# zhengyk19/vit-rpe-rope

Hardware: AMD Instinct MI355X
Metric: train images/sec, CIFAR-10 ViT d=192 L=6 H=6 (higher is better)
Workload: dtype bf16; 1 GPU; CIFAR-10-shaped 32x32 patch4 ViT d=192 L=6 H=6, --pos_encoding rope-axial theta=100, bf16, full train step (fwd+CE+bwd+AdamW), random-init weights; per_gpu_batch=512, global_batch=512, parallelism=dp1, hip_graph=True

## Files before the change

include/vitpe_debug.h:

```cpp
#ifndef VITPE_DEBUG_H
#define VITPE_DEBUG_H
#include "vitpe.h"
#ifdef __cplusplus
extern "C" {
#endif

int vitpe_selftest_mma(int dtype, const void* A, const void* Bt, const void* Brow, float* C_row,
                       float* C_tr, vitpe_stream_t stream);

int vitpe_debug_attn_occupancy(int which);
int vitpe_debug_wgrad_census(int dtype, const vitpe_wgrad_problem* problems, int nprob, unsigned long long* census,
                             vitpe_stream_t stream);
int vitpe_debug_attn_census(const void* xn, const void* wqkv, void* out, const float* cos, const float* sin,
                            int B, unsigned long long* census, vitpe_stream_t stream);
int vitpe_debug_attn32_census(const void* xn, const void* wqkv_wide, void* out, const float* cos, const float* sin,
                              int B, unsigned long long* census, int exp, vitpe_stream_t stream);
int vitpe_debug_tail2_census(const void* attn_out, const void* x_in, const void* Wp_packed, const float* bp,
                             const float* gamma, const float* beta, void* x_mid, float* mean2, float* rstd2,
                             void* xn_out, const void* W1_packed, const float* b1, const void* W2_packed,
                             const float* b2, void* gp_out, void* h_out, void* out, float* mean_out, float* rstd_out,
                             int M, int HID, unsigned long long* census, int exp, vitpe_stream_t stream);
int vitpe_debug_set_gemm2d_mt(int mt);
int vitpe_debug_set_wgrad_wide(int on);
int vitpe_debug_read_bw(const void* src, long long bytes, int depth, int workgroups, unsigned* sink, vitpe_stream_t stream);
#ifdef __cplusplus
}
#endif
#endif
```

vit-rpe-rope_amd/csrc/attn.hip:

```cpp
#include "attn_common.h"
#include <stdlib.h>
#include <type_traits>

namespace vitpe {

template <typename T, typename C, int KM, int NTH = 384>
VITPE_DEV void stage_tokens(const AttnArgs& a, int b, T* xs, T* hbuf, int hbuf_elems, float* s_tab, float* s_coef,
                            int tid, int nthreads, bool stage_tables) {
  constexpr int CHN = CH<T>::n;
  constexpr int DCH = C::LDX / CHN;
  constexpr int D = C::DD;
  const int N = C::ntok(a);
  const T* xg = reinterpret_cast<const T*>(a.xn) + (size_t)b * N * D;
  const Chunk16 zero = {0u, 0u, 0u, 0u};
  constexpr int TOTAL = C::NP * DCH;
  constexpr int ITERS = (TOTAL + NTH - 1) / NTH;
  Chunk16 v[ITERS];
#pragma unroll
  for (int it = 0; it < ITERS; ++it) {
    const int q = tid + it * nthreads, row = q / DCH, cc = q % DCH;
    v[it] = zero;
    if (q < TOTAL && row < N && cc * CHN < D) v[it] = *reinterpret_cast<const Chunk16*>(xg + (size_t)row * D + cc * CHN);
  }
  if (a.ln_gamma != nullptr) {
// ... 340 lines not shown
    f32x4 o[NT];
#pragma unroll
    for (int dt = 0; dt < NT; ++dt) o[dt] = z4;
#pragma unroll
    for (int sc = 0; sc < SC; ++sc) {
      const Frag<T> bp = acc_to_frag<T>(s[2 * sc], (2 * sc + 1 < MT) ? s[(2 * sc + 1 < MT) ? 2 * sc + 1 : 0] : z4);
#pragma unroll
      for (int dt = 0; dt < NT; ++dt) mma(vf[dt][sc], bp, o[dt]);
    }
    const float inv = __builtin_amdgcn_rcpf(l);
    if (sizeof(T) == 2) {
#pragma unroll
      for (int dp = 0; dp < NT; dp += 2) {
        uint32_t lo[2], hi[2];
#pragma unroll
        for (int w2 = 0; w2 < 2; ++w2) {
          bf16x2 pa, pb;
          const f32x4 oa = o[dp] * inv, ob = o[dp + 1] * inv;
          pa[0] = (bf16)oa[2 * w2]; pa[1] = (bf16)oa[2 * w2 + 1];
          pb[0] = (bf16)ob[2 * w2]; pb[1] = (bf16)ob[2 * w2 + 1];
          const auto r = __builtin_amdgcn_permlane16_swap(__builtin_bit_cast(uint32_t, pa), __builtin_bit_cast(uint32_t, pb),
                                                         false, false);
          lo[w2] = r[0]; hi[w2] = r[1];
        }
        const int f0 = 16 * (dp + (g & 1)) + 8 * (g >> 1);
        if (it < MT - 1 || i < N)
          *reinterpret_cast<Chunk16*>(outp + (size_t)i * D + f0) = (Chunk16){lo[0], lo[1], hi[0], hi[1]};
      }
    } else if (it < MT - 1 || i < N) {
#pragma unroll
      for (int dt = 0; dt < NT; ++dt)
        st4(outp + (size_t)i * D + 16 * dt + 4 * g, o[dt][0] * inv, o[dt][1] * inv, o[dt][2] * inv, o[dt][3] * inv);
    }
  }
  stamp(6);
}

template <typename T, typename C, int NTH>
VITPE_DEV void stage_rows_plain(const T* src, T* dst, int ld, int N, int tid) {
  constexpr int CHN = CH<T>::n, D = C::DD, CPRW = D / CHN, RPP = NTH / CPRW, ITERS = C::NP / RPP;
  const int cc = tid % CPRW, r0 = tid / CPRW;
  const Chunk16 zero = {0u, 0u, 0u, 0u};
  Chunk16 v[ITERS];
#pragma unroll
  for (int it = 0; it < ITERS; ++it) {
    const int row = r0 + it * RPP;
    v[it] = *reinterpret_cast<const Chunk16*>(src + (size_t)min(row, N - 1) * D + cc * CHN);
    if (row >= N) v[it] = zero;
  }
#pragma unroll
  for (int it = 0; it < ITERS; ++it) *reinterpret_cast<Chunk16*>(dst + (r0 + it * RPP) * ld + cc * CHN) = v[it];
}

template <int HD, int D, int MT, int KM, int NTOK, int IPW, bool LNF, bool MIXED, int PDEG = 7>
__global__ __launch_bounds__(64 * (D / HD) * IPW, 3) void attn_bwd_reg_kernel(AttnArgs a) {
  using T = bf16;
  using C = AttnCfg<T, HD, D, MT, 1, NTOK>;
  constexpr int NT = C::NT, KS = C::KS, HC = C::HC, SC = C::SC, NTH = 64 * C::H;
  static_assert(NT == 2 && HC == 1, "head dimension 32");
  constexpr int CSLD = HD / 2 + 8;
  constexpr int FRAG = 64 * 8;
  constexpr int XS_ELEMS = IPW * C::NP * C::LDX, DOS_ELEMS = IPW * C::H * MT * FRAG;
  __shared__ __attribute__((aligned(16))) T xs_all[XS_ELEMS > DOS_ELEMS ? XS_ELEMS : DOS_ELEMS];
  __shared__ __attribute__((aligned(16))) T qs_all[IPW * C::H * MT * FRAG];
  __shared__ __attribute__((aligned(16))) float s_tab[KM == KM_RELATIVE ? C::H * C::TABLD : 4];
  __shared__ __attribute__((aligned(16))) float s_coef[KM == KM_POLY ? C::PESZ : 4];
  __shared__ __attribute__((aligned(16))) float s_cos[KM == KM_ROPE ? C::NP * CSLD : 4];
  __shared__ __attribute__((aligned(16))) float s_sin[KM == KM_ROPE ? C::NP * CSLD : 4];
  __shared__ __attribute__((aligned(16))) float s_stat[IPW * C::H * 2 * C::NP];
  __shared__ float s_dtab[KM == KM_RELATIVE ? C::H * C::TABLD : 4];
  __shared__ float s_dcoef[C::H * (C::MAXDEG + 1)];
  __shared__ float s_dfreq[2 * C::H * (HD / 2)];

  const int N = C::ntok(a), P = N - 1;
  const int lane = threadIdx.x & 63;
  const int wave_all = __builtin_amdgcn_readfirstlane(threadIdx.x >> 6);
  const int img = wave_all / C::H, h = wave_all % C::H;
  const int b_raw = blockIdx.x * IPW + img;
  const bool live = b_raw < a.B;
  const int b = live ? b_raw : a.B - 1;
  const int tid_img = threadIdx.x % NTH;
  T* const xs = xs_all + img * C::NP * C::LDX;
  T* const qsw = qs_all + wave_all * MT * FRAG + lane * 8;
  T* const dsw = xs_all + wave_all * MT * FRAG + lane * 8;
  float* const lse_w = s_stat + (img * C::H + h) * 2 * C::NP;
  float* const del_w = lse_w + C::NP;
  float* const dtab_i = s_dtab;
  float* const dcoef_i = s_dcoef;
  float* const dfreq_i = s_dfreq;
  const int c = lane & 15, g = lane >> 4;
  const f32x4 z4 = {0.f, 0.f, 0.f, 0.f};
  constexpr bool mixed = (KM == KM_ROPE) && MIXED;

  const T* const Wh = reinterpret_cast<const T*>(a.wqkv) + ((size_t)h * 3 * NT * KS * 64 + lane) * 8;
  auto wload = [&](Frag<T> (&w)[NT][KS], int mat) {
#pragma unroll
    for (int nt = 0; nt < NT; ++nt)
#pragma unroll
      for (int ks = 0; ks < KS; ++ks) w[nt][ks] = ld_frag(Wh + (size_t)((mat * NT + nt) * KS + ks) * 64 * 8);
  };
  Frag<T> w[NT][KS];
  wload(w, 2);
  stage_tokens_fwd<T, C, KM, NTH, LNF>(a, b, xs, s_tab, s_coef, tid_img, false, IPW == 1 || img == 0);
  if (KM == KM_ROPE && !mixed) {
    constexpr int F4 = HD / 8;
    for (int q = threadIdx.x; q < C::NP * F4; q += NTH * IPW) {
      const int f4 = q % F4, row = q / F4;
      f32x4 cv = {1.f, 1.f, 1.f, 1.f}, sv = {0.f, 0.f, 0.f, 0.f};
      if (row >= 1 && row < N) {
        cv = *reinterpret_cast<const f32x4*>(a.cos + (size_t)(row - 1) * (HD / 2) + 4 * f4);
        sv = *reinterpret_cast<const f32x4*>(a.sin + (size_t)(row - 1) * (HD / 2) + 4 * f4);
      }
      *reinterpret_cast<f32x4*>(&s_cos[row * CSLD + 4 * f4]) = cv;
      *reinterpret_cast<f32x4*>(&s_sin[row * CSLD + 4 * f4]) = sv;
    }
  }
  if (KM == KM_RELATIVE)
    for (int q = threadIdx.x; q < C::H * C::TABLD; q += NTH * IPW) s_dtab[q] = 0.f;
  for (int q = threadIdx.x; q < C::H * (C::MAXDEG + 1); q += NTH * IPW) s_dcoef[q] = 0.f;
  for (int q = threadIdx.x; q < 2 * C::H * (HD / 2); q += NTH * IPW) s_dfreq[q] = 0.f;
  __syncthreads();

  const T* const xrow = xs + c * C::LDX + 8 * g;
  const unsigned hoff = mixed ? (unsigned)(h * P * (HD / 2)) : 0u;
  auto cs_vec = [&](int tok, int f, f32x4& cv, f32x4& sv) {
    if (!mixed) {
      cv = *reinterpret_cast<const f32x4*>(&s_cos[tok * CSLD + f]);
      sv = *reinterpret_cast<const f32x4*>(&s_sin[tok * CSLD + f]);
    } else {
      const bool ok = tok >= 1 && tok < N;
      const unsigned o = hoff + (unsigned)((min(max(tok, 1), N - 1) - 1) * (HD / 2) + f);
      const f32x4 cg = *reinterpret_cast<const f32x4*>(a.cos + o), sg = *reinterpret_cast<const f32x4*>(a.sin + o);
      cv = ok ? cg : (f32x4){1.f, 1.f, 1.f, 1.f};
      sv = ok ? sg : z4;
    }
  };
  auto proj_sw = [&](int tt, bool rope, float sc, Frag<T>& dst) {
    Frag<T> xf[KS];
#pragma unroll
    for (int ks = 0; ks < KS; ++ks) xf[ks] = ld_frag(xrow + 16 * tt * C::LDX + 32 * ks);
    __builtin_amdgcn_sched_barrier(0);
    f32x4 acc[NT] = {z4, z4};
#pragma unroll
    for (int ks = 0; ks < KS; ++ks)
#pragma unroll
      for (int nt = 0; nt < NT; ++nt) mma(w[nt][ks], xf[ks], acc[nt]);
    __builtin_amdgcn_sched_barrier(0);
    if (KM == KM_ROPE && rope) {
      f32x4 cv, sv;
      cs_vec(16 * tt + c, 4 * g, cv, sv);
      const f32x4 x1 = acc[0], x2 = acc[1];
      acc[0] = x1 * cv - x2 * sv;
      acc[1] = x1 * sv + x2 * cv;
    }
    dst = acc_to_frag<T>(acc[0] * sc, acc[1] * sc);
    asm volatile("" : "+v"(dst.v));
  };
  Frag<T> e0, e1;
#pragma unroll
  for (int t = 0; t < 8; ++t) {
    e0.v[t] = (bf16)((t < 4 && 4 * g + t == c) ? 1.0f : 0.0f);
    e1.v[t] = (bf16)((t >= 4 && 4 * g + t - 4 == c) ? 1.0f : 0.0f);
  }
  auto transpose_pair = [&](const Frag<T>& fa, const Frag<T>* fb, Frag<T>& d0, Frag<T>& d1) {
    f32x4 a0 = z4, a1 = z4, b0 = z4, b1 = z4;
    mma(fa, e0, a0);
    mma(fa, e1, a1);
    if (fb != nullptr) { mma(*fb, e0, b0); mma(*fb, e1, b1); }
    d0 = acc_to_frag<T>(a0, b0);
    d1 = acc_to_frag<T>(a1, b1);
  };

  const float qsc = a.scale * LOG2E;
  Frag<T> vkf[MT], kf[MT];
#pragma unroll
  for (int tt = 0; tt < MT; ++tt) proj_sw(tt, false, 1.0f, vkf[tt]);
  wload(w, 1);
  __builtin_amdgcn_sched_barrier(0);
#pragma unroll
  for (int tt = 0; tt < MT; ++tt) proj_sw(tt, true, 1.0f, kf[tt]);
  wload(w, 0);
  __builtin_amdgcn_sched_barrier(0);
#pragma unroll
  for (int tt = 0; tt < MT; ++tt) {
    Frag<T> qf;
    proj_sw(tt, true, qsc, qf);
    *reinterpret_cast<bf16x8*>(qsw + tt * FRAG) = qf.v;
  }
  __syncthreads();
  if (!live) return;
  {
    const T* dog = reinterpret_cast<const T*>(a.dout) + (size_t)b * N * D + h * HD;
    Frag<T> df[MT];
#pragma unroll
    for (int tt = 0; tt < MT; ++tt) {
      const int tok = 16 * tt + c;
      bf16x4 lo = {(bf16)0.f, (bf16)0.f, (bf16)0.f, (bf16)0.f}, hi = lo;
      if (tok < N) {
        lo = *reinterpret_cast<const bf16x4*>(dog + (size_t)tok * D + 4 * g);
        hi = *reinterpret_cast<const bf16x4*>(dog + (size_t)tok * D + 16 + 4 * g);
      }
      df[tt].v = __builtin_shufflevector(lo, hi, 0, 1, 2, 3, 4, 5, 6, 7);
    }
#pragma unroll
    for (int tt = 0; tt < MT; ++tt) *reinterpret_cast<bf16x8*>(dsw + tt * FRAG) = df[tt].v;
  }
  auto qf_load = [&](int tt) { Frag<T> f; f.v = *reinterpret_cast<const bf16x8*>(qsw + tt * FRAG); return f; };
  auto dof_load = [&](int tt) { Frag<T> f; f.v = *reinterpret_cast<const bf16x8*>(dsw + tt * FRAG); return f; };
  Frag<T> ktf[NT][SC];
#pragma unroll
  for (int scx = 0; scx < SC; ++scx)
    transpose_pair(kf[2 * scx], (2 * scx + 1 < MT) ? &kf[(2 * scx + 1 < MT) ? 2 * scx + 1 : 0] : nullptr, ktf[0][scx], ktf[1][scx]);

  T* const dqg = reinterpret_cast<T*>(a.out) + (size_t)b * N * 3 * D + h * HD;
  auto store_pair = [&](T* rowp, const f32x4& o0, const f32x4& o1, bool ok) {
    uint32_t lo[2], hi[2];
#pragma unroll
    for (int w2 = 0; w2 < 2; ++w2) {
      bf16x2 pa, pb;
      pa[0] = (bf16)o0[2 * w2]; pa[1] = (bf16)o0[2 * w2 + 1];
      pb[0] = (bf16)o1[2 * w2]; pb[1] = (bf16)o1[2 * w2 + 1];
      const auto r = __builtin_amdgcn_permlane16_swap(__builtin_bit_cast(uint32_t, pa), __builtin_bit_cast(uint32_t, pb), false, false);
      lo[w2] = r[0]; hi[w2] = r[1];
    }
    const int f0 = 16 * (g & 1) + 8 * (g >> 1);
    if (ok) *reinterpret_cast<Chunk16*>(rowp + f0) = (Chunk16){lo[0], lo[1], hi[0], hi[1]};
  };

  float cacc[PDEG + 1];
#pragma unroll
  for (int k = 0; k <= PDEG; ++k) cacc[k] = 0.f;
#pragma unroll
  for (int it = 0; it < MT; ++it) {
    __builtin_amdgcn_sched_barrier(0);
    const int i = 16 * it + c;
    const Frag<T> dof = dof_load(it), qfi = qf_load(it);
    f32x4 s[MT], dp[MT];
    float m = -1e30f;
    typedef __attribute__((ext_vector_type(4))) unsigned u32x4;
    const unsigned xyi = (KM == KM_POLY) ? reinterpret_cast<const unsigned*>(s_coef + C::H * C::PBLD)[i] : 0u;
    const float* const ptab = s_coef + (a.coeff_per_head ? h : 0) * C::PBLD;
    const bool qcls = (it == 0) && (c == 0);
#pragma unroll
    for (int jt = 0; jt < MT; ++jt) {
      s[jt] = z4;
      mma(kf[jt], qfi, s[jt]);
      dp[jt] = z4;
      mma(vkf[jt], dof, dp[jt]);
      const u32x4 xyj = (KM == KM_POLY) ? *reinterpret_cast<const u32x4*>(s_coef + C::H * C::PBLD + 16 * jt + 4 * g) : (u32x4){0u, 0u, 0u, 0u};
#pragma unroll
      for (int r = 0; r < 4; ++r) {
        const int j = 16 * jt + 4 * g + r;
        float v = s[jt][r];
        if (KM == KM_RELATIVE) v += pe_bias2<C, KM>(a, s_tab, s_coef, h, i, j, N);
        if (KM == KM_POLY) {
          const float bv = ptab[__builtin_amdgcn_sad_u8(xyi, xyj[r], 0u)];
          const bool cls = qcls || (jt == 0 && r == 0 && g == 0);
          v += cls ? 0.f : bv;
        }
        if (jt == MT - 1) v = (j < N) ? v : -1e30f;
        s[jt][r] = v;
        m = fmaxf(m, v);
      }
    }
    m = xg_max(m);
    float l = 0.f;
#pragma unroll
    for (int jt = 0; jt < MT; ++jt)
#pragma unroll
      for (int r = 0; r < 4; ++r) { const float p = __builtin_amdgcn_exp2f(s[jt][r] - m); s[jt][r] = p; l += p; }
    l = xg_sum(l);
    const float inv = __builtin_amdgcn_rcpf(l);
    float dl = 0.f;
#pragma unroll
    for (int jt = 0; jt < MT; ++jt)
#pragma unroll
      for (int r = 0; r < 4; ++r) { s[jt][r] *= inv; dl += s[jt][r] * dp[jt][r]; }
    dl = xg_sum(dl);
    if (g == 0) { lse_w[i] = m + __builtin_amdgcn_logf(l); del_w[i] = dl; }
    const bool qvalid = (it < MT - 1) || (i < N);
    float tacc[PDEG + 1];
#pragma unroll
    for (int k = 0; k <= PDEG; ++k) tacc[k] = 0.f;
#pragma unroll
    for (int jt = 0; jt < MT; ++jt) {
      if (KM == KM_POLY) __builtin_amdgcn_sched_barrier(0);
      const u32x4 xyj = (KM == KM_POLY) ? *reinterpret_cast<const u32x4*>(s_coef + C::H * C::PBLD + 16 * jt + 4 * g) : (u32x4){0u, 0u, 0u, 0u};
#pragma unroll
      for (int r = 0; r < 4; ++r) {
        const int j = 16 * jt + 4 * g + r;
        const bool valid = qvalid && ((jt < MT - 1) || (j < N));
        const float ds = valid ? s[jt][r] * (dp[jt][r] - dl) : 0.f;
        dp[jt][r] = ds;
        if (KM == KM_POLY) {
          const float dsk = (jt == 0 && r == 0) ? (g == 0 ? 0.f : ds) : ds;
          const float x = (float)__builtin_amdgcn_sad_u8(xyi, xyj[r], 0u);
          float pw = x;
          tacc[0] += dsk;
#pragma unroll
          for (int k = 1; k <= PDEG; ++k) { tacc[k] = fmaf(dsk, pw, tacc[k]); if (k < PDEG) pw *= x; }
        }
      }
    }
    if (KM == KM_POLY) {
      const float qm = (it == 0 && c == 0) ? 0.f : 1.f;
#pragma unroll
      for (int k = 0; k <= PDEG; ++k) {
        cacc[k] = fmaf(qm, tacc[k], cacc[k]);
        asm volatile("" : "+v"(cacc[k]));
      }
    }
    if (KM == KM_RELATIVE) {
#pragma unroll
      for (int jt = 0; jt < MT; ++jt) {
        float d0, d1;
        tile_diag_sums(dp[jt], lane, d0, d1);
        const int idx0 = 16 * (it - jt) + c + N - 1;
        if (g == 0) {
          if (idx0 >= 0 && idx0 <= 2 * N - 2) atomicAdd(&dtab_i[h * C::TABLD + idx0], d0);
          if (c >= 1 && idx0 - 16 >= 0 && idx0 - 16 <= 2 * N - 2) atomicAdd(&dtab_i[h * C::TABLD + idx0 - 16], d1);
        }
      }
    }
    f32x4 dqa[NT] = {z4, z4};
#pragma unroll
    for (int scx = 0; scx < SC; ++scx) {
      const Frag<T> bs = acc_to_frag<T>(dp[2 * scx], (2 * scx + 1 < MT) ? dp[(2 * scx + 1 < MT) ? 2 * scx + 1 : 0] : z4);
#pragma unroll
      for (int dt = 0; dt < NT; ++dt) mma(ktf[dt][scx], bs, dqa[dt]);
    }
    if (mixed) {
      const bool tok_ok = i >= 1 && i < N;
      f32x4 dph;
#pragma unroll
      for (int r = 0; r < 4; ++r) dph[r] = dqa[1][r] * (float)qfi.v[r] - dqa[0][r] * (float)qfi.v[4 + r];
      mixed_freq_grad_tile(dfreq_i, dph, i, tok_ok, 16 * it, h, C::H, P, a.grid, HD / 2, 4 * g, LN2, lane);
    }
    if (KM == KM_ROPE) {
      f32x4 cv, sv;
      cs_vec(min(i, C::NP - 1), 4 * g, cv, sv);
      const f32x4 d1 = dqa[0], d2 = dqa[1];
      dqa[0] = d1 * cv + d2 * sv;
      dqa[1] = d2 * cv - d1 * sv;
    }
    store_pair(dqg + (size_t)i * 3 * D, dqa[0] * a.scale, dqa[1] * a.scale, qvalid);
  }

  if (KM == KM_POLY) {
#pragma unroll
    for (int k = 0; k <= PDEG; ++k)
      if (k <= a.degree) {
        const float t = wave_sum(cacc[k]);
        if (lane == 0) atomicAdd(&dcoef_i[(a.coeff_per_head ? h : 0) * (C::MAXDEG + 1) + k], t);
      }
  }
  Frag<T> qtf[NT][SC], dotf[NT][SC];
  __builtin_amdgcn_sched_barrier(0);
#pragma unroll
  for (int scx = 0; scx < SC; ++scx) {
    const bool two = 2 * scx + 1 < MT;
    const Frag<T> qa = qf_load(2 * scx), qb = qf_load(two ? 2 * scx + 1 : 0);
    transpose_pair(qa, two ? &qb : nullptr, qtf[0][scx], qtf[1][scx]);
    const Frag<T> da = dof_load(2 * scx), db = dof_load(two ? 2 * scx + 1 : 0);
    transpose_pair(da, two ? &db : nullptr, dotf[0][scx], dotf[1][scx]);
  }
  __builtin_amdgcn_s_waitcnt(0xC07F);

#pragma unroll
  for (int jt = 0; jt < MT; ++jt) {
    __builtin_amdgcn_sched_barrier(0);
    const int j = 16 * jt + c;
    const bool kvalid = (jt < MT - 1) || (j < N);
    const unsigned xyk = (KM == KM_POLY) ? reinterpret_cast<const unsigned*>(s_coef + C::H * C::PBLD)[j] : 0u;
    const float* const ptab2 = s_coef + (a.coeff_per_head ? h : 0) * C::PBLD;
    const bool kcls = (jt == 0) && (c == 0);
    f32x4 p[MT], ds[MT];
#pragma unroll
    for (int it = 0; it < MT; ++it) {
      const Frag<T> dof = dof_load(it), qfi = qf_load(it);
      p[it] = z4;
      mma(qfi, kf[jt], p[it]);
      ds[it] = z4;
      mma(dof, vkf[jt], ds[it]);
      const f32x4 lse = *reinterpret_cast<const f32x4*>(&lse_w[16 * it + 4 * g]);
      const f32x4 dlv = *reinterpret_cast<const f32x4*>(&del_w[16 * it + 4 * g]);
      typedef __attribute__((ext_vector_type(4))) unsigned u32x4;
      const u32x4 xyq = (KM == KM_POLY) ? *reinterpret_cast<const u32x4*>(s_coef + C::H * C::PBLD + 16 * it + 4 * g) : (u32x4){0u, 0u, 0u, 0u};
#pragma unroll
      for (int r = 0; r < 4; ++r) {
        const int i = 16 * it + 4 * g + r;
        float sv = p[it][r];
        if (KM == KM_RELATIVE) sv += pe_bias2<C, KM>(a, s_tab, s_coef, h, i, j, N);
        if (KM == KM_POLY) {
          const float bv = ptab2[__builtin_amdgcn_sad_u8(xyk, xyq[r], 0u)];
          const bool cls = kcls || (it == 0 && r == 0 && g == 0);
          sv += cls ? 0.f : bv;
        }
        const bool valid = kvalid && ((it < MT - 1) || (i < N));
        const float pv = valid ? __builtin_amdgcn_exp2f(sv - lse[r]) : 0.f;
        p[it][r] = pv;
        ds[it][r] = pv * (ds[it][r] - dlv[r]);
      }
    }
    f32x4 dva[NT] = {z4, z4}, dka[NT] = {z4, z4};
#pragma unroll
    for (int scx = 0; scx < SC; ++scx) {
      const bool two = (2 * scx + 1 < MT);
      const Frag<T> bp = acc_to_frag<T>(p[2 * scx], two ? p[two ? 2 * scx + 1 : 0] : z4);
      const Frag<T> bs = acc_to_frag<T>(ds[2 * scx], two ? ds[two ? 2 * scx + 1 : 0] : z4);
#pragma unroll
      for (int dt = 0; dt < NT; ++dt) {
        mma(dotf[dt][scx], bp, dva[dt]);
        mma(qtf[dt][scx], bs, dka[dt]);
      }
    }
    dka[0] *= LN2; dka[1] *= LN2;
    if (mixed) {
      const bool tok_ok = j >= 1 && j < N;
      f32x4 dph;
#pragma unroll
      for (int r = 0; r < 4; ++r) dph[r] = dka[1][r] * (float)kf[jt].v[r] - dka[0][r] * (float)kf[jt].v[4 + r];
      mixed_freq_grad_tile(dfreq_i, dph, j, tok_ok, 16 * jt, h, C::H, P, a.grid, HD / 2, 4 * g, 1.0f, lane);
    }
    if (KM == KM_ROPE) {
      f32x4 cv, sv;
      cs_vec(min(j, C::NP - 1), 4 * g, cv, sv);
      const f32x4 d1 = dka[0], d2 = dka[1];
      dka[0] = d1 * cv + d2 * sv;
      dka[1] = d2 * cv - d1 * sv;
    }
    store_pair(dqg + (size_t)j * 3 * D + D, dka[0], dka[1], kvalid);
    store_pair(dqg + (size_t)j * 3 * D + 2 * D, dva[0], dva[1], kvalid);
  }

  __syncthreads();
  const int nrun = NTH * min(IPW, a.B - (int)blockIdx.x * IPW);
  if (KM == KM_RELATIVE) {
    for (int q = threadIdx.x; q < C::H * (2 * N - 1); q += nrun) {
      const int hh = q / (2 * N - 1), i = q % (2 * N - 1);
      atomicAdd(a.dtable + q, s_dtab[hh * C::TABLD + i]);
    }
  } else if (KM == KM_POLY) {
    const int nh = a.coeff_per_head ? C::H : 1;
    for (int q = threadIdx.x; q < nh * (a.degree + 1); q += nrun) {
      const int hh = q / (a.degree + 1), k = q % (a.degree + 1);
      atomicAdd(a.dcoeff + q, s_dcoef[hh * (C::MAXDEG + 1) + k]);
    }
  } else if (mixed) {
    for (int q = threadIdx.x; q < 2 * C::H * (HD / 2); q += nrun) atomicAdd(a.dfreqs + q, s_dfreq[q]);
  }
}

template <typename T, int HD, int D, int MT, int HPP, int KM, int NTOK>
__global__ __launch_bounds__(384) void attn_bwd_kernel(AttnArgs a) {
  using C = AttnCfg<T, HD, D, MT, HPP, NTOK>;
  __shared__ __attribute__((aligned(16))) T xs[C::NP * C::LDX];
  __shared__ __attribute__((aligned(16))) T hb[4 * HPP * C::HSZ];
  __shared__ __attribute__((aligned(16))) float s_tab[KM == KM_RELATIVE ? C::H * C::TABLD : 4];
  __shared__ __attribute__((aligned(16))) float s_coef[KM == KM_POLY ? C::PESZ : 4];
  __shared__ __attribute__((aligned(16))) float s_stat[HPP * 2 * C::NP];
  __shared__ float s_dtab[KM == KM_RELATIVE ? C::H * C::TABLD : 4];
  __shared__ float s_dcoef[C::H * (C::MAXDEG + 1)];
  __shared__ float s_dfreq[2 * C::H * (HD / 2)];
  constexpr int SLD = HPP * HD + Pad<T>::elems;
  __shared__ __attribute__((aligned(16))) T s_dq[3 * C::NP * SLD];

  const int N = C::ntok(a);
  const int b = blockIdx.x;
  const int lane = threadIdx.x & 63;
  const int wave = __builtin_amdgcn_readfirstlane(threadIdx.x >> 6);
  const int c = lane & 15, g = lane >> 4;
  const int P = N - 1;
  WFrags<T, C> wf;
  {
    const int hh = wave / 3, mat = wave % 3;
    if (hh < HPP && hh < C::H) load_w<T, C>(a, wf, hh, mat, lane);
  }
  stage_tokens<T, C, KM>(a, b, xs, hb, 4 * HPP * C::HSZ, s_tab, s_coef, threadIdx.x, 384, true);
  if (KM == KM_RELATIVE)
    for (int q = threadIdx.x; q < C::H * C::TABLD; q += 384) s_dtab[q] = 0.f;
  for (int q = threadIdx.x; q < C::H * (C::MAXDEG + 1); q += 384) s_dcoef[q] = 0.f;
  for (int q = threadIdx.x; q < 2 * C::H * (HD / 2); q += 384) s_dfreq[q] = 0.f;
  __syncthreads();

  constexpr int CHN = CH<T>::n;
// ... 257 lines not shown
            *reinterpret_cast<const Chunk16*>(s_dq + (mat * C::NP + row) * SLD + cc * CHN);
      }
    }
  }

  if (KM == KM_RELATIVE) {
    for (int q = threadIdx.x; q < C::H * (2 * N - 1); q += 384) {
      const int h = q / (2 * N - 1), i = q % (2 * N - 1);
      atomicAdd(a.dtable + q, s_dtab[h * C::TABLD + i]);
    }
  } else if (KM == KM_POLY) {
    const int nh = a.coeff_per_head ? C::H : 1;
    for (int q = threadIdx.x; q < nh * (a.degree + 1); q += 384) {
      const int h = q / (a.degree + 1), k = q % (a.degree + 1);
      atomicAdd(a.dcoeff + q, s_dcoef[h * (C::MAXDEG + 1) + k]);
    }
  } else if (mixed) {
    for (int q = threadIdx.x; q < 2 * C::H * (HD / 2); q += 384) atomicAdd(a.dfreqs + q, s_dfreq[q]);
  }
}

template <typename T>
__global__ void pack_qkv_kernel(const float* __restrict__ w, T* __restrict__ dst, int D, int HD) {
  const int NT = HD / 16, KS = D / 32, H = D / HD;
  const long long total = (long long)3 * D * D;
  for (long long idx = (long long)blockIdx.x * blockDim.x + threadIdx.x; idx < total;
       idx += (long long)gridDim.x * blockDim.x) {
    const int e = (int)(idx & 7), l = (int)((idx >> 3) & 63);
    long long blk = idx >> 9;
    const int ks = (int)(blk % KS); blk /= KS;
    const int nt = (int)(blk % NT); blk /= NT;
    const int mat = (int)(blk % 3);
    const int h = (int)(blk / 3);
    if (h >= H) continue;
    const int c = l & 15, g = l >> 4;
    dst[idx] = from_f32<T>(w[(size_t)(mat * D + h * HD + 16 * nt + c) * D + 32 * ks + 8 * g + e]);
  }
}

}

using namespace vitpe;

extern "C" int vitpe_pack_qkv_weights(int dtype, const float* wqkv, void* packed, int D, int HD, hipStream_t stream) {
  VITPE_REQUIRE(wqkv && packed && D > 0 && HD > 0 && D % HD == 0 && HD % 16 == 0 && D % 32 == 0);
  VITPE_REQUIRE(dtype == 0 || dtype == 1);
  const long long total = (long long)3 * D * D;
  const unsigned blocks = (unsigned)min((total + 255) / 256, (long long)2048);
  if (dtype == 1) hipLaunchKernelGGL(pack_qkv_kernel<bf16>, dim3(blocks), dim3(256), 0, stream, wqkv, (bf16*)packed, D, HD);
  else hipLaunchKernelGGL(pack_qkv_kernel<float>, dim3(blocks), dim3(256), 0, stream, wqkv, (float*)packed, D, HD);
  VITPE_CHECK_LAUNCH();
}

template <typename T, int HD, int D, int MT, int HPP, int KM, int NTOK>
static int launch_attn3(bool bwd, const AttnArgs& a, hipStream_t s) {
  constexpr bool REG_BWD = sizeof(T) == 2 && D / HD <= 6;
  if constexpr (REG_BWD) {
    if (bwd) {
      const dim3 grid((a.B + 1) / 2), block(64 * (D / HD) * 2);
      const bool ln = a.ln_gamma != nullptr;
      if constexpr (KM == KM_ROPE) {
        if (a.mode == PE_ROPE_MIXED) {
          if (ln) hipLaunchKernelGGL((attn_bwd_reg_kernel<HD, D, MT, KM, NTOK, 2, true, true>), grid, block, 0, s, a);
          else hipLaunchKernelGGL((attn_bwd_reg_kernel<HD, D, MT, KM, NTOK, 2, false, true>), grid, block, 0, s, a);
          VITPE_CHECK_LAUNCH();
        }
      }
      if constexpr (KM == KM_POLY) {
        if (a.degree <= 3) {
          if (ln) hipLaunchKernelGGL((attn_bwd_reg_kernel<HD, D, MT, KM, NTOK, 2, true, false, 3>), grid, block, 0, s, a);
          else hipLaunchKernelGGL((attn_bwd_reg_kernel<HD, D, MT, KM, NTOK, 2, false, false, 3>), grid, block, 0, s, a);
          VITPE_CHECK_LAUNCH();
        }
      }
      if (ln) hipLaunchKernelGGL((attn_bwd_reg_kernel<HD, D, MT, KM, NTOK, 2, true, false>), grid, block, 0, s, a);
      else hipLaunchKernelGGL((attn_bwd_reg_kernel<HD, D, MT, KM, NTOK, 2, false, false>), grid, block, 0, s, a);
      VITPE_CHECK_LAUNCH();
    }
  }
  if (bwd) {
    if constexpr (!REG_BWD) hipLaunchKernelGGL((attn_bwd_kernel<T, HD, D, MT, HPP, KM, NTOK>), dim3(a.B), dim3(384), 0, s, a);
  } else {
    constexpr int IPW = (sizeof(T) == 2 && D / HD <= 6) ? 2 : 1;
    const dim3 grid((a.B + IPW - 1) / IPW), block(64 * (D / HD) * IPW);
    if (a.ln_gamma != nullptr) hipLaunchKernelGGL((attn_fwd_kernel<T, HD, D, MT, KM, NTOK, IPW, true>), grid, block, 0, s, a);
    else hipLaunchKernelGGL((attn_fwd_kernel<T, HD, D, MT, KM, NTOK, IPW, false>), grid, block, 0, s, a);
  }
  VITPE_CHECK_LAUNCH();
}

template <typename T, int HD, int D, int MT, int HPP, int NTOK>
static int launch_attn2(bool bwd, const AttnArgs& a, hipStream_t s) {
  switch (a.mode) {
    case PE_RELATIVE: return launch_attn3<T, HD, D, MT, HPP, KM_RELATIVE, NTOK>(bwd, a, s);
    case PE_POLY: return launch_attn3<T, HD, D, MT, HPP, KM_POLY, NTOK>(bwd, a, s);
    case PE_ROPE_AXIAL:
    case PE_ROPE_MIXED: return launch_attn3<T, HD, D, MT, HPP, KM_ROPE, NTOK>(bwd, a, s);
    default: return launch_attn3<T, HD, D, MT, HPP, KM_PLAIN, NTOK>(bwd, a, s);
  }
}

template <typename T, int HD, int D, int MT, int HPP>
static int launch_attn(bool bwd, const AttnArgs& a, hipStream_t s) {
  if (a.N == 65) return launch_attn2<T, HD, D, MT, HPP, 65>(bwd, a, s);
  return launch_attn2<T, HD, D, MT, HPP, 0>(bwd, a, s);
}

static int dispatch_attn(bool bwd, int dtype, int D, int HD, const AttnArgs& a, hipStream_t s) {
  const int MT = (a.N + 15) / 16;
  if (HD != 32 || MT != 5) return (int)hipErrorNotSupported;
  if (dtype == 1) {
    if (D == 192) return launch_attn<bf16, 32, 192, 5, 2>(bwd, a, s);
    if (D == 96) return launch_attn<bf16, 32, 96, 5, 2>(bwd, a, s);
// ... 97 lines not shown
```

vit-rpe-rope_amd/vitpe/kernels.py:

```python
from __future__ import annotations

import ctypes
from typing import Optional, Tuple

import torch

from . import _lib as L
from ._lib import check, dtype_code, lib, ptr, require_device, stream_ptr

SPLITS_TARGET_WGS = 512


def _f32(t, name):
    if t is not None and t.dtype != torch.float32:
        raise L.VitpeError(f"{name} must be float32")


def gemm_nt(a, w, bias=None, epi=L.EPI_BIAS, resid=None, u=None, out=None):
    require_device(a, w, bias, resid, u, out)
    M, K = a.shape
    N = w.shape[0]
    assert w.shape[1] == K and a.dtype == w.dtype
    _f32(bias, "bias")
    c = out if out is not None else torch.empty((M, N), dtype=a.dtype, device=a.device)
# ... 333 lines not shown
    HD = D // num_heads
    assert wqkv.numel() == 3 * D * D and wqkv.dtype == xn.dtype
    o = out if out is not None else torch.empty_like(xn)
    name, lnp = _ln_variant("vitpe_fused_attention_fwd", ln)
    if ln is not None:
        lnp += (ptr(xn_out),)
    check(getattr(lib(), name)(dtype_code(xn.dtype), ptr(xn), *lnp, ptr(wqkv), ptr(o), B, N, D, HD, *_pe_tail(pe),
                               stream_ptr()), name)
    return o


def fused_attention_wide_supported(dtype, N, D, HD) -> bool:
    return bool(lib().vitpe_fused_attention_wide_supported(dtype_code(dtype), N, D, HD))


def pack_qkv_weights_wide(wqkv_f32, dtype, num_heads, out=None):
    require_device(wqkv_f32, out)
    _f32(wqkv_f32, "wqkv")
    D = wqkv_f32.shape[1]
    n = lib().vitpe_qkv_wide_pack_elems(D)
    o = out if out is not None else torch.empty(n, dtype=dtype, device=wqkv_f32.device)
    assert o.numel() == n and o.dtype == dtype
    check(lib().vitpe_pack_qkv_weights_wide(dtype_code(dtype), ptr(wqkv_f32), ptr(o), D, D // num_heads, stream_ptr()),
          "vitpe_pack_qkv_weights_wide")
    return o


def fused_attention_fwd_wide(xn, wqkv_wide, num_heads, pe: PETables, out=None, ln=None, xn_out=None):
    require_device(xn, wqkv_wide, pe.cos, pe.sin, pe.table, pe.coeff, out, xn_out)
    B, N, D = xn.shape
    HD = D // num_heads
    assert wqkv_wide.numel() == 3 * D * D and wqkv_wide.dtype == xn.dtype
    o = out if out is not None else torch.empty_like(xn)
    g = ln if ln is not None else (None, None, None, None)
    if ln is not None:
        require_device(*ln)
    check(lib().vitpe_fused_attention_fwd_wide(dtype_code(xn.dtype), ptr(xn), ptr(g[0]), ptr(g[1]), ptr(g[2]), ptr(g[3]),
                                               ptr(xn_out), ptr(wqkv_wide), ptr(o), B, N, D, HD, *_pe_tail(pe),
                                               stream_ptr()), "vitpe_fused_attention_fwd_wide")
    return o


def fused_attention_bwd(xn, wqkv, dout, num_heads, pe: PETables, dtable=None, dcoeff=None, dfreqs=None, out=None, ln=None):
    require_device(xn, wqkv, dout, dtable, dcoeff, dfreqs, out)
    B, N, D = xn.shape
    HD = D // num_heads
    dqkv = out if out is not None else torch.empty((B, N, 3 * D), dtype=xn.dtype, device=xn.device)
    name, lnp = _ln_variant("vitpe_fused_attention_bwd", ln)
    check(getattr(lib(), name)(dtype_code(xn.dtype), ptr(xn), *lnp, ptr(wqkv), ptr(dout), ptr(dqkv), B, N, D, HD,
                               *_pe_tail(pe), ptr(dtable), ptr(dcoeff), ptr(dfreqs), stream_ptr()), name)
    return dqkv


def attention_core_supported(dtype, N, HD):
    return bool(lib().vitpe_attention_core_supported(dtype_code(dtype), N, HD))


def attention_core_fwd(qkv, num_heads, pe: PETables, out=None):
    require_device(qkv, out)
    B, N, D3 = qkv.shape
    D = D3 // 3
    HD = D // num_heads
    o = out if out is not None else torch.empty((B, N, D), dtype=qkv.dtype, device=qkv.device)
    check(lib().vitpe_attention_core_fwd(dtype_code(qkv.dtype), ptr(qkv), ptr(o), B, N, num_heads, HD, *_pe_tail(pe),
                                         stream_ptr()), "vitpe_attention_core_fwd")
    return o


def attention_core_probs(qkv, num_heads, pe: PETables, cls_only=False, out=None):
    require_device(qkv, out, pe.cos, pe.sin, pe.table, pe.coeff)
    B, N, D3 = qkv.shape
    HD = D3 // 3 // num_heads
    shape = (B, num_heads, N) if cls_only else (B, num_heads, N, N)
    o = out if out is not None else torch.empty(shape, dtype=torch.float32, device=qkv.device)
    if tuple(o.shape) != shape or o.dtype != torch.float32:
        raise L.VitpeError(f"attention_core_probs: out must be float32 {shape}")
    check(lib().vitpe_attention_core_probs(dtype_code(qkv.dtype), ptr(qkv), ptr(o), int(bool(cls_only)), B, N, num_heads, HD,
                                           *_pe_tail(pe), stream_ptr()), "vitpe_attention_core_probs")
    return o


def attention_fused64_supported(dtype, N, num_heads, HD) -> bool:
    return bool(lib().vitpe_attention_fused64_supported(dtype_code(dtype), int(N), int(num_heads), int(HD)))


def attention_fused64_fwd(xn, wqkv_pk, num_heads, pe: PETables, qkv_out=None, out=None):
    require_device(xn, wqkv_pk, qkv_out, out, pe.cos, pe.sin, pe.table, pe.coeff)
    B, N, D = xn.shape
    HD = D // num_heads
    assert wqkv_pk.numel() == 3 * D * D and wqkv_pk.dtype == xn.dtype
    if qkv_out is not None:
        assert qkv_out.shape == (B, N, 3 * D) and qkv_out.dtype == xn.dtype and qkv_out.is_contiguous()
    o = out if out is not None else torch.empty_like(xn)
    check(lib().vitpe_attention_fused64_fwd(dtype_code(xn.dtype), ptr(xn), ptr(wqkv_pk), ptr(qkv_out), ptr(o), B, N, num_heads,
                                            HD, *_pe_tail(pe), stream_ptr()), "vitpe_attention_fused64_fwd")
    return o


def attention_core_bwd(qkv, dout, num_heads, pe: PETables, dtable=None, dcoeff=None, dfreqs=None, out=None,
                       dcos=None, dsin=None):
    require_device(qkv, dout, dtable, dcoeff, dfreqs, out, dcos, dsin)
    B, N, D3 = qkv.shape
    HD = D3 // 3 // num_heads
    dqkv = out if out is not None else torch.empty_like(qkv)
    if dcos is None and dsin is None:
        check(lib().vitpe_attention_core_bwd(dtype_code(qkv.dtype), ptr(qkv), ptr(dout), ptr(dqkv), B, N, num_heads, HD,
# ... 514 lines not shown
```

Before: 366,100 images/sec.

## Handle 65th token separately in attention backward to skip padded tile

Adds an ODD variant of the register attention backward kernel for 65-token sequences. The first 64 tokens run through the existing 16x16 MFMA tiles, and the lone 65th token gets its own row/column path using DPP row reductions and small shared-memory staging, so the mostly padded fifth tile is no longer processed. The variant is enabled by default for plain and non-mixed rope modes. The trade is extra special-case code, more shared-memory traffic for the odd row, and some rounding points that differ from the tiled path.

```diff
diff --git a/include/vitpe_debug.h b/include/vitpe_debug.h
--- a/include/vitpe_debug.h
+++ b/include/vitpe_debug.h
@@ -22,6 +22,7 @@
                              int M, int HID, unsigned long long* census, int exp, vitpe_stream_t stream);
 int vitpe_debug_set_gemm2d_mt(int mt);
 int vitpe_debug_set_wgrad_wide(int on);
+int vitpe_debug_set_attn_bwd_odd(int on);
 int vitpe_debug_read_bw(const void* src, long long bytes, int depth, int workgroups, unsigned* sink, vitpe_stream_t stream);
 #ifdef __cplusplus
 }
diff --git a/vit-rpe-rope_amd/csrc/attn.hip b/vit-rpe-rope_amd/csrc/attn.hip
--- a/vit-rpe-rope_amd/csrc/attn.hip
+++ b/vit-rpe-rope_amd/csrc/attn.hip
@@ -416,12 +416,31 @@
   for (int it = 0; it < ITERS; ++it) *reinterpret_cast<Chunk16*>(dst + (r0 + it * RPP) * ld + cc * CHN) = v[it];
 }
 
-template <int HD, int D, int MT, int KM, int NTOK, int IPW, bool LNF, bool MIXED, int PDEG = 7>
+#define VITPE_ROW_DPP(v, ctrl) __builtin_bit_cast(float, __builtin_amdgcn_update_dpp(0, __builtin_bit_cast(int, (v)), (ctrl), 0xF, 0xF, true))
+VITPE_DEV float row16_all_max(float v) {
+  v = fmaxf(v, VITPE_ROW_DPP(v, 0xB1));
+  v = fmaxf(v, VITPE_ROW_DPP(v, 0x4E));
+  v = fmaxf(v, VITPE_ROW_DPP(v, 0x124));
+  return fmaxf(v, VITPE_ROW_DPP(v, 0x128));
+}
+VITPE_DEV float row16_all_sum(float v) {
+  v += VITPE_ROW_DPP(v, 0xB1);
+  v += VITPE_ROW_DPP(v, 0x4E);
+  v += VITPE_ROW_DPP(v, 0x124);
+  return v + VITPE_ROW_DPP(v, 0x128);
+}
+
+template <int HD, int D, int MT, int KM, int NTOK, int IPW, bool LNF, bool MIXED, int PDEG = 7, bool ODD = false>
 __global__ __launch_bounds__(64 * (D / HD) * IPW, 3) void attn_bwd_reg_kernel(AttnArgs a) {
   using T = bf16;
   using C = AttnCfg<T, HD, D, MT, 1, NTOK>;
-  constexpr int NT = C::NT, KS = C::KS, HC = C::HC, SC = C::SC, NTH = 64 * C::H;
+  constexpr int NT = C::NT, KS = C::KS, HC = C::HC, NTH = 64 * C::H;
   static_assert(NT == 2 && HC == 1, "head dimension 32");
+  static_assert(!ODD || (NTOK == 65 && MT == 5 && (KM == KM_PLAIN || (KM == KM_ROPE && !MIXED))), "64 + 1 mapping");
+  constexpr int MTL = ODD ? MT - 1 : MT;
+  constexpr int SC = (MTL + 1) / 2;
+  constexpr int OTOK = 16 * (MT - 1);
+  constexpr int OT = ODD ? MT - 1 : 0;
   constexpr int CSLD = HD / 2 + 8;
   constexpr int FRAG = 64 * 8;
   constexpr int XS_ELEMS = IPW * C::NP * C::LDX, DOS_ELEMS = IPW * C::H * MT * FRAG;
@@ -447,6 +466,10 @@
   T* const xs = xs_all + img * C::NP * C::LDX;
   T* const qsw = qs_all + wave_all * MT * FRAG + lane * 8;
   T* const dsw = xs_all + wave_all * MT * FRAG + lane * 8;
+  float* const ocp = reinterpret_cast<float*>(xs_all + (wave_all * MT + MT - 1) * FRAG);
+  float* const ocs = ocp + 64;
+  float* const ors = ocp + 128;
+  T* const odo = reinterpret_cast<T*>(ocp + 192);
   float* const lse_w = s_stat + (img * C::H + h) * 2 * C::NP;
   float* const del_w = lse_w + C::NP;
   float* const dtab_i = s_dtab;
@@ -500,9 +523,11 @@
     }
   };
   auto proj_sw = [&](int tt, bool rope, float sc, Frag<T>& dst) {
+    const bool odd = ODD && tt == MTL;
+    const T* const xp = odd ? xs + OTOK * C::LDX + 8 * g : xrow + 16 * tt * C::LDX;
     Frag<T> xf[KS];
 #pragma unroll
-    for (int ks = 0; ks < KS; ++ks) xf[ks] = ld_frag(xrow + 16 * tt * C::LDX + 32 * ks);
+    for (int ks = 0; ks < KS; ++ks) xf[ks] = ld_frag(xp + 32 * ks);
     __builtin_amdgcn_sched_barrier(0);
     f32x4 acc[NT] = {z4, z4};
 #pragma unroll
@@ -512,7 +537,7 @@
     __builtin_amdgcn_sched_barrier(0);
     if (KM == KM_ROPE && rope) {
       f32x4 cv, sv;
-      cs_vec(16 * tt + c, 4 * g, cv, sv);
+      cs_vec(odd ? OTOK : 16 * tt + c, 4 * g, cv, sv);
       const f32x4 x1 = acc[0], x2 = acc[1];
       acc[0] = x1 * cv - x2 * sv;
       acc[1] = x1 * sv + x2 * cv;
@@ -558,7 +583,7 @@
     Frag<T> df[MT];
 #pragma unroll
     for (int tt = 0; tt < MT; ++tt) {
-      const int tok = 16 * tt + c;
+      const int tok = (ODD && tt == MTL) ? OTOK : 16 * tt + c;
       bf16x4 lo = {(bf16)0.f, (bf16)0.f, (bf16)0.f, (bf16)0.f}, hi = lo;
       if (tok < N) {
         lo = *reinterpret_cast<const bf16x4*>(dog + (size_t)tok * D + 4 * g);
@@ -567,14 +592,20 @@
       df[tt].v = __builtin_shufflevector(lo, hi, 0, 1, 2, 3, 4, 5, 6, 7);
     }
 #pragma unroll
-    for (int tt = 0; tt < MT; ++tt) *reinterpret_cast<bf16x8*>(dsw + tt * FRAG) = df[tt].v;
+    for (int tt = 0; tt < MTL; ++tt) *reinterpret_cast<bf16x8*>(dsw + tt * FRAG) = df[tt].v;
+    if (ODD && c == 0) *reinterpret_cast<bf16x8*>(odo + 8 * g) = df[MTL].v;
   }
   auto qf_load = [&](int tt) { Frag<T> f; f.v = *reinterpret_cast<const bf16x8*>(qsw + tt * FRAG); return f; };
   auto dof_load = [&](int tt) { Frag<T> f; f.v = *reinterpret_cast<const bf16x8*>(dsw + tt * FRAG); return f; };
+  auto odof_load = [&]() { Frag<T> f; f.v = *reinterpret_cast<const bf16x8*>(odo + 8 * g); return f; };
+  auto row_frag = [&](const float* row, int scx) {
+    return acc_to_frag<T>(*reinterpret_cast<const f32x4*>(row + 32 * scx + 4 * g),
+                          *reinterpret_cast<const f32x4*>(row + 32 * scx + 16 + 4 * g));
+  };
   Frag<T> ktf[NT][SC];
 #pragma unroll
   for (int scx = 0; scx < SC; ++scx)
-    transpose_pair(kf[2 * scx], (2 * scx + 1 < MT) ? &kf[(2 * scx + 1 < MT) ? 2 * scx + 1 : 0] : nullptr, ktf[0][scx], ktf[1][scx]);
+    transpose_pair(kf[2 * scx], (2 * scx + 1 < MTL) ? &kf[(2 * scx + 1 < MTL) ? 2 * scx + 1 : 0] : nullptr, ktf[0][scx], ktf[1][scx]);
 
   T* const dqg = reinterpret_cast<T*>(a.out) + (size_t)b * N * 3 * D + h * HD;
   auto store_pair = [&](T* rowp, const f32x4& o0, const f32x4& o1, bool ok) {
@@ -595,18 +626,26 @@
 #pragma unroll
   for (int k = 0; k <= PDEG; ++k) cacc[k] = 0.f;
 #pragma unroll
-  for (int it = 0; it < MT; ++it) {
+  for (int it = 0; it < MTL; ++it) {
     __builtin_amdgcn_sched_barrier(0);
     const int i = 16 * it + c;
     const Frag<T> dof = dof_load(it), qfi = qf_load(it);
-    f32x4 s[MT], dp[MT];
+    f32x4 s[MTL], dp[MTL];
     float m = -1e30f;
     typedef __attribute__((ext_vector_type(4))) unsigned u32x4;
     const unsigned xyi = (KM == KM_POLY) ? reinterpret_cast<const unsigned*>(s_coef + C::H * C::PBLD)[i] : 0u;
     const float* const ptab = s_coef + (a.coeff_per_head ? h : 0) * C::PBLD;
     const bool qcls = (it == 0) && (c == 0);
-#pragma unroll
-    for (int jt = 0; jt < MT; ++jt) {
+    float so = 0.f, dpo = 0.f;
+    if (ODD) {
+      f32x4 t0 = z4, t1 = z4;
+      mma(kf[OT], qfi, t0);
+      mma(vkf[OT], dof, t1);
+      so = t0[0];
+      dpo = t1[0];
+    }
+#pragma unroll
+    for (int jt = 0; jt < MTL; ++jt) {
       s[jt] = z4;
       mma(kf[jt], qfi, s[jt]);
       dp[jt] = z4;
@@ -622,38 +661,47 @@
           const bool cls = qcls || (jt == 0 && r == 0 && g == 0);
           v += cls ? 0.f : bv;
         }
-        if (jt == MT - 1) v = (j < N) ? v : -1e30f;
+        if (!ODD && jt == MT - 1) v = (j < N) ? v : -1e30f;
         s[jt][r] = v;
         m = fmaxf(m, v);
       }
     }
     m = xg_max(m);
+    if (ODD) m = fmaxf(m, so);
     float l = 0.f;
 #pragma unroll
-    for (int jt = 0; jt < MT; ++jt)
+    for (int jt = 0; jt < MTL; ++jt)
 #pragma unroll
       for (int r = 0; r < 4; ++r) { const float p = __builtin_amdgcn_exp2f(s[jt][r] - m); s[jt][r] = p; l += p; }
     l = xg_sum(l);
+    if (ODD) { so = __builtin_amdgcn_exp2f(so - m); l += so; }
     const float inv = __builtin_amdgcn_rcpf(l);
     float dl = 0.f;
 #pragma unroll
-    for (int jt = 0; jt < MT; ++jt)
+    for (int jt = 0; jt < MTL; ++jt)
 #pragma unroll
       for (int r = 0; r < 4; ++r) { s[jt][r] *= inv; dl += s[jt][r] * dp[jt][r]; }
     dl = xg_sum(dl);
+    if (ODD) { so *= inv; dl = fmaf(so, dpo, dl); }
     if (g == 0) { lse_w[i] = m + __builtin_amdgcn_logf(l); del_w[i] = dl; }
-    const bool qvalid = (it < MT - 1) || (i < N);
+    float dso = 0.f;
+    if (ODD) {
+      dso = so * (dpo - dl);
+      if (g == 0) { ocp[i] = so; ocs[i] = dso; }
+      dso = (float)(bf16)dso;
+    }
+    const bool qvalid = ODD || (it < MT - 1) || (i < N);
     float tacc[PDEG + 1];
 #pragma unroll
     for (int k = 0; k <= PDEG; ++k) tacc[k] = 0.f;
 #pragma unroll
-    for (int jt = 0; jt < MT; ++jt) {
+    for (int jt = 0; jt < MTL; ++jt) {
       if (KM == KM_POLY) __builtin_amdgcn_sched_barrier(0);
       const u32x4 xyj = (KM == KM_POLY) ? *reinterpret_cast<const u32x4*>(s_coef + C::H * C::PBLD + 16 * jt + 4 * g) : (u32x4){0u, 0u, 0u, 0u};
 #pragma unroll
       for (int r = 0; r < 4; ++r) {
         const int j = 16 * jt + 4 * g + r;
-        const bool valid = qvalid && ((jt < MT - 1) || (j < N));
+        const bool valid = qvalid && (ODD || (jt < MT - 1) || (j < N));
         const float ds = valid ? s[jt][r] * (dp[jt][r] - dl) : 0.f;
         dp[jt][r] = ds;
         if (KM == KM_POLY) {
@@ -676,7 +724,7 @@
     }
     if (KM == KM_RELATIVE) {
 #pragma unroll
-      for (int jt = 0; jt < MT; ++jt) {
+      for (int jt = 0; jt < MTL; ++jt) {
         float d0, d1;
         tile_diag_sums(dp[jt], lane, d0, d1);
         const int idx0 = 16 * (it - jt) + c + N - 1;
@@ -689,9 +737,16 @@
     f32x4 dqa[NT] = {z4, z4};
 #pragma unroll
     for (int scx = 0; scx < SC; ++scx) {
-      const Frag<T> bs = acc_to_frag<T>(dp[2 * scx], (2 * scx + 1 < MT) ? dp[(2 * scx + 1 < MT) ? 2 * scx + 1 : 0] : z4);
+      const Frag<T> bs = acc_to_frag<T>(dp[2 * scx], (2 * scx + 1 < MTL) ? dp[(2 * scx + 1 < MTL) ? 2 * scx + 1 : 0] : z4);
 #pragma unroll
       for (int dt = 0; dt < NT; ++dt) mma(ktf[dt][scx], bs, dqa[dt]);
+    }
+    if (ODD) {
+#pragma unroll
+      for (int r = 0; r < 4; ++r) {
+        dqa[0][r] = fmaf(dso, (float)kf[OT].v[r], dqa[0][r]);
+        dqa[1][r] = fmaf(dso, (float)kf[OT].v[4 + r], dqa[1][r]);
+      }
     }
     if (mixed) {
       const bool tok_ok = i >= 1 && i < N;
@@ -718,11 +773,74 @@
         if (lane == 0) atomicAdd(&dcoef_i[(a.coeff_per_head ? h : 0) * (C::MAXDEG + 1) + k], t);
       }
   }
+  float pr[MTL], dsr[MTL];
+  float poo = 0.f, dsoo = 0.f;
+  Frag<T> qfo, dofo;
+  if constexpr (ODD) {
+    __builtin_amdgcn_sched_barrier(0);
+    qfo = qf_load(OT);
+    dofo = odof_load();
+    float m = -1e30f, dpr[MTL];
+#pragma unroll
+    for (int jt = 0; jt < MTL; ++jt) {
+      f32x4 t0 = z4, t1 = z4;
+      mma(qfo, kf[jt], t0);
+      mma(dofo, vkf[jt], t1);
+      pr[jt] = t0[0];
+      dpr[jt] = t1[0];
+      m = fmaxf(m, pr[jt]);
+    }
+    f32x4 t0 = z4, t1 = z4;
+    mma(qfo, kf[OT], t0);
+    mma(dofo, vkf[OT], t1);
+    m = fmaxf(row16_all_max(m), t0[0]);
+    float l = 0.f;
+#pragma unroll
+    for (int jt = 0; jt < MTL; ++jt) { pr[jt] = __builtin_amdgcn_exp2f(pr[jt] - m); l += pr[jt]; }
+    poo = __builtin_amdgcn_exp2f(t0[0] - m);
+    l = row16_all_sum(l) + poo;
+    const float inv = __builtin_amdgcn_rcpf(l);
+    float dl = 0.f;
+#pragma unroll
+    for (int jt = 0; jt < MTL; ++jt) { pr[jt] *= inv; dl = fmaf(pr[jt], dpr[jt], dl); }
+    poo *= inv;
+    dl = fmaf(poo, t1[0], row16_all_sum(dl));
+#pragma unroll
+    for (int jt = 0; jt < MTL; ++jt) {
+      dsr[jt] = pr[jt] * (dpr[jt] - dl);
+      if (g == 0) ors[16 * jt + c] = dsr[jt];
+      pr[jt] = (float)(bf16)pr[jt];
+      dsr[jt] = (float)(bf16)dsr[jt];
+    }
+    dsoo = (float)(bf16)(poo * (t1[0] - dl));
+    poo = (float)(bf16)poo;
+    __builtin_amdgcn_s_waitcnt(0xC07F);
+    f32x4 dqa[NT] = {z4, z4};
+#pragma unroll
+    for (int scx = 0; scx < SC; ++scx) {
+      const Frag<T> bs = row_frag(ors, scx);
+#pragma unroll
+      for (int dt = 0; dt < NT; ++dt) mma(ktf[dt][scx], bs, dqa[dt]);
+    }
+#pragma unroll
+    for (int r = 0; r < 4; ++r) {
+      dqa[0][r] = fmaf(dsoo, (float)kf[OT].v[r], dqa[0][r]);
+      dqa[1][r] = fmaf(dsoo, (float)kf[OT].v[4 + r], dqa[1][r]);
+    }
+    if (KM == KM_ROPE) {
+      f32x4 cv, sv;
+      cs_vec(OTOK, 4 * g, cv, sv);
+      const f32x4 d1 = dqa[0], d2 = dqa[1];
+      dqa[0] = d1 * cv + d2 * sv;
+      dqa[1] = d2 * cv - d1 * sv;
+    }
+    store_pair(dqg + (size_t)OTOK * 3 * D, dqa[0] * a.scale, dqa[1] * a.scale, c == 0);
+  }
   Frag<T> qtf[NT][SC], dotf[NT][SC];
   __builtin_amdgcn_sched_barrier(0);
 #pragma unroll
   for (int scx = 0; scx < SC; ++scx) {
-    const bool two = 2 * scx + 1 < MT;
+    const bool two = 2 * scx + 1 < MTL;
     const Frag<T> qa = qf_load(2 * scx), qb = qf_load(two ? 2 * scx + 1 : 0);
     transpose_pair(qa, two ? &qb : nullptr, qtf[0][scx], qtf[1][scx]);
     const Frag<T> da = dof_load(2 * scx), db = dof_load(two ? 2 * scx + 1 : 0);
@@ -731,16 +849,16 @@
   __builtin_amdgcn_s_waitcnt(0xC07F);
 
 #pragma unroll
-  for (int jt = 0; jt < MT; ++jt) {
+  for (int jt = 0; jt < MTL; ++jt) {
     __builtin_amdgcn_sched_barrier(0);
     const int j = 16 * jt + c;
-    const bool kvalid = (jt < MT - 1) || (j < N);
+    const bool kvalid = ODD || (jt < MT - 1) || (j < N);
     const unsigned xyk = (KM == KM_POLY) ? reinterpret_cast<const unsigned*>(s_coef + C::H * C::PBLD)[j] : 0u;
     const float* const ptab2 = s_coef + (a.coeff_per_head ? h : 0) * C::PBLD;
     const bool kcls = (jt == 0) && (c == 0);
-    f32x4 p[MT], ds[MT];
-#pragma unroll
-    for (int it = 0; it < MT; ++it) {
+    f32x4 p[MTL], ds[MTL];
+#pragma unroll
+    for (int it = 0; it < MTL; ++it) {
       const Frag<T> dof = dof_load(it), qfi = qf_load(it);
       p[it] = z4;
       mma(qfi, kf[jt], p[it]);
@@ -760,7 +878,7 @@
           const bool cls = kcls || (it == 0 && r == 0 && g == 0);
           sv += cls ? 0.f : bv;
         }
-        const bool valid = kvalid && ((it < MT - 1) || (i < N));
+        const bool valid = kvalid && (ODD || (it < MT - 1) || (i < N));
         const float pv = valid ? __builtin_amdgcn_exp2f(sv - lse[r]) : 0.f;
         p[it][r] = pv;
         ds[it][r] = pv * (ds[it][r] - dlv[r]);
@@ -769,13 +887,22 @@
     f32x4 dva[NT] = {z4, z4}, dka[NT] = {z4, z4};
 #pragma unroll
     for (int scx = 0; scx < SC; ++scx) {
-      const bool two = (2 * scx + 1 < MT);
+      const bool two = (2 * scx + 1 < MTL);
       const Frag<T> bp = acc_to_frag<T>(p[2 * scx], two ? p[two ? 2 * scx + 1 : 0] : z4);
       const Frag<T> bs = acc_to_frag<T>(ds[2 * scx], two ? ds[two ? 2 * scx + 1 : 0] : z4);
 #pragma unroll
       for (int dt = 0; dt < NT; ++dt) {
         mma(dotf[dt][scx], bp, dva[dt]);
         mma(qtf[dt][scx], bs, dka[dt]);
+      }
+    }
+    if constexpr (ODD) {
+#pragma unroll
+      for (int r = 0; r < 4; ++r) {
+        dva[0][r] = fmaf(pr[jt], (float)dofo.v[r], dva[0][r]);
+        dva[1][r] = fmaf(pr[jt], (float)dofo.v[4 + r], dva[1][r]);
+        dka[0][r] = fmaf(dsr[jt], (float)qfo.v[r], dka[0][r]);
+        dka[1][r] = fmaf(dsr[jt], (float)qfo.v[4 + r], dka[1][r]);
       }
     }
     dka[0] *= LN2; dka[1] *= LN2;
@@ -795,6 +922,36 @@
     }
     store_pair(dqg + (size_t)j * 3 * D + D, dka[0], dka[1], kvalid);
     store_pair(dqg + (size_t)j * 3 * D + 2 * D, dva[0], dva[1], kvalid);
+  }
+  if constexpr (ODD) {
+    __builtin_amdgcn_sched_barrier(0);
+    f32x4 dva[NT] = {z4, z4}, dka[NT] = {z4, z4};
+#pragma unroll
+    for (int scx = 0; scx < SC; ++scx) {
+      const Frag<T> bp = row_frag(ocp, scx), bs = row_frag(ocs, scx);
+#pragma unroll
+      for (int dt = 0; dt < NT; ++dt) {
+        mma(dotf[dt][scx], bp, dva[dt]);
+        mma(qtf[dt][scx], bs, dka[dt]);
+      }
+    }
+#pragma unroll
+    for (int r = 0; r < 4; ++r) {
+      dva[0][r] = fmaf(poo, (float)dofo.v[r], dva[0][r]);
+      dva[1][r] = fmaf(poo, (float)dofo.v[4 + r], dva[1][r]);
+      dka[0][r] = fmaf(dsoo, (float)qfo.v[r], dka[0][r]);
+      dka[1][r] = fmaf(dsoo, (float)qfo.v[4 + r], dka[1][r]);
+    }
+    dka[0] *= LN2; dka[1] *= LN2;
+    if (KM == KM_ROPE) {
+      f32x4 cv, sv;
+      cs_vec(OTOK, 4 * g, cv, sv);
+      const f32x4 d1 = dka[0], d2 = dka[1];
+      dka[0] = d1 * cv + d2 * sv;
+      dka[1] = d2 * cv - d1 * sv;
+    }
+    store_pair(dqg + (size_t)OTOK * 3 * D + D, dka[0], dka[1], c == 0);
+    store_pair(dqg + (size_t)OTOK * 3 * D + 2 * D, dva[0], dva[1], c == 0);
   }
 
   __syncthreads();
@@ -1158,6 +1315,9 @@
   VITPE_CHECK_LAUNCH();
 }
 
+static bool g_bwd_odd = true;
+extern "C" int vitpe_debug_set_attn_bwd_odd(int on) { g_bwd_odd = on != 0; return 0; }
+
 template <typename T, int HD, int D, int MT, int HPP, int KM, int NTOK>
 static int launch_attn3(bool bwd, const AttnArgs& a, hipStream_t s) {
   constexpr bool REG_BWD = sizeof(T) == 2 && D / HD <= 6;
@@ -1165,6 +1325,13 @@
     if (bwd) {
       const dim3 grid((a.B + 1) / 2), block(64 * (D / HD) * 2);
       const bool ln = a.ln_gamma != nullptr;
+      if constexpr (NTOK == 65 && (KM == KM_PLAIN || KM == KM_ROPE)) {
+        if (g_bwd_odd && a.mode != PE_ROPE_MIXED) {
+          if (ln) hipLaunchKernelGGL((attn_bwd_reg_kernel<HD, D, MT, KM, NTOK, 2, true, false, 7, true>), grid, block, 0, s, a);
+          else hipLaunchKernelGGL((attn_bwd_reg_kernel<HD, D, MT, KM, NTOK, 2, false, false, 7, true>), grid, block, 0, s, a);
+          VITPE_CHECK_LAUNCH();
+        }
+      }
       if constexpr (KM == KM_ROPE) {
         if (a.mode == PE_ROPE_MIXED) {
           if (ln) hipLaunchKernelGGL((attn_bwd_reg_kernel<HD, D, MT, KM, NTOK, 2, true, true>), grid, block, 0, s, a);
diff --git a/vit-rpe-rope_amd/vitpe/kernels.py b/vit-rpe-rope_amd/vitpe/kernels.py
--- a/vit-rpe-rope_amd/vitpe/kernels.py
+++ b/vit-rpe-rope_amd/vitpe/kernels.py
@@ -409,6 +409,10 @@
     return dqkv
 
 
+def debug_set_attn_bwd_odd(on: bool):
+    check(L.debug_lib().vitpe_debug_set_attn_bwd_odd(1 if on else 0), "vitpe_debug_set_attn_bwd_odd")
+
+
 def attention_core_supported(dtype, N, HD):
     return bool(lib().vitpe_attention_core_supported(dtype_code(dtype), N, HD))
 
```

After: 364,500 images/sec. No clear change (-0.4%).
